# jinbeizame007/pytorch-r2d2-DPG

Hardware: NVIDIA H100
Metric: learner sequence-steps/sec (batch x seq_len) (higher is better)
Workload: dtype bf16x3 (fp32 operands split into bf16 hi+lo, three tensor-core passes, fp32 accumulate: ~16-bit operands)

## Files before the change

### include/r2d2_b200.h

```cpp
#ifndef R2D2_B200_H_
#define R2D2_B200_H_

#include <stddef.h>
#include <stdint.h>

#ifdef __cplusplus
extern "C" {
#endif

#define R2D2_OK 0
#define R2D2_ERR_CUDA (-1)
#define R2D2_ERR_ARG (-2)
#define R2D2_ERR_UNSUPPORTED (-3)
#define R2D2_ERR_STATE (-4)

typedef void* r2d2_stream_t;

int r2d2_version(void);
long long r2d2_launch_count(void);
const char* r2d2_arch(void);
const char* r2d2_last_error(void);
int r2d2_device_sm_count(int* out);

int r2d2_gemm_f32(int layout, int M, int N, int K, const float* A, long long lda, const float* B, long long ldb,
// ... 13 lines not shown

int r2d2_lstm_net_forward(const r2d2_net_shape* shape, const float* params, const float* obs, const float* act,
                          const float* h0, const float* c0, int T, int B, int repeat, int head_first_row,
                          float* out, float* workspace, r2d2_stream_t stream);

int r2d2_lstm_net_backward(const r2d2_net_shape* shape, const float* params, const float* obs, const float* act,
                           const float* d_out, int T, int B, int repeat, int head_first_row, float* grads,
                           float* d_act, float* workspace, r2d2_stream_t stream);

int r2d2_lstm_scan_forward(const float* gin, const float* whh, const float* h0, const float* c0, float* gates,
                           float* hs, float* cs, float* head_in, int T, int B, int H, int repeat, float* scratch,
                           r2d2_stream_t stream);
int r2d2_lstm_scan_backward(const float* gates, const float* hs, const float* cs, const float* whh,
                            const float* dh_head, int head_first_step, float* dgates, float* dgin, int T, int B,
                            int H, int repeat, float* scratch, r2d2_stream_t stream);

int r2d2_set_gemm_impl(int impl);
int r2d2_get_gemm_impl(void);
int r2d2_set_scan_impl(int impl);
int r2d2_get_scan_impl(void);
int r2d2_scan_status(int* status, r2d2_stream_t stream);

int r2d2_td_priority(const float* q, const float* q_next, const float* rew, const float* term, int L, int B,
                     int A, int burn_in, int n_step, float gamma, float eta, float* target, float* dq,
                     float* td_sq, float* priority, float* critic_loss, r2d2_stream_t stream);
int r2d2_td_priority_weighted(const float* q, const float* q_next, const float* rew, const float* term,
                              const float* is_weight, int L, int B, int A, int burn_in, int n_step, float gamma, float eta,
                              float* target, float* dq, float* td_sq, float* priority, float* critic_loss,
                              r2d2_stream_t stream);

#define R2D2_RESCALE_REFERENCE 0
#define R2D2_RESCALE_INVERTIBLE 1
#define R2D2_PRIORITY_SQUARED 0
#define R2D2_PRIORITY_ABS 1
typedef struct {
// ... 189 lines not shown
```

### pytorch-r2d2-dpg_b200/csrc/api.cu

```cuda
#include <atomic>
#include <cmath>

#include "common.cuh"
#include "elementwise.cuh"
#include "gemm.cuh"
#include "learner.cuh"
#include "lstm_scan.cuh"
#include "net.cuh"
#include "policy.cuh"
#include "replay.cuh"
#include "td3.cuh"

namespace r2d2 {
static thread_local std::string g_last_error;
static std::atomic<long long> g_launches{0};
void set_last_error(const std::string& msg) { g_last_error = msg; }
const char* last_error() { return g_last_error.c_str(); }
void count_launch(int n) { g_launches.fetch_add(n, std::memory_order_relaxed); }
long long launch_count() { return g_launches.load(std::memory_order_relaxed); }
int num_sms() {
  static std::atomic<int> cache[64];
  int dev = 0;
  if (cudaGetDevice(&dev) != cudaSuccess || dev < 0 || dev >= 64) return 132;
  int n = cache[dev].load(std::memory_order_relaxed);
// ... 99 lines not shown
  ScanFwdParams p;
  p.gin = gin; p.whh = whh; p.h0 = h0; p.c0 = c0; p.gates = gates; p.hs = hs; p.cs = cs; p.head_in = head_in;
  p.T = T; p.B = B; p.H = H; p.repeat = repeat; p.scratch = scratch;
  return lstm_scan_forward(p, S(stream));
}

int r2d2_lstm_scan_backward(const float* gates, const float* hs, const float* cs, const float* whh,
                            const float* dh_head, int head_first_step, float* dgates, float* dgin, int T, int B,
                            int H, int repeat, float* scratch, r2d2_stream_t stream) {
  ScanBwdParams p;
  p.gates = gates; p.hs = hs; p.cs = cs; p.whh = whh; p.dh_head = dh_head; p.head_first_step = head_first_step;
  p.dgates = dgates; p.dgin = dgin; p.T = T; p.B = B; p.H = H; p.repeat = repeat; p.scratch = scratch;
  return lstm_scan_backward(p, S(stream));
}

int r2d2_set_gemm_impl(int impl) {
  gemm_set_impl(impl != 0);
  gemm_set_impl_skinny_mma(impl != 2);
  return R2D2_OK;
}
int r2d2_get_gemm_impl(void) { return gemm_get_impl(); }
int r2d2_set_scan_impl(int impl) { lstm_scan_set_impl(impl); return R2D2_OK; }
int r2d2_get_scan_impl(void) { return lstm_scan_get_impl(); }
int r2d2_scan_status(int* status, r2d2_stream_t stream) { return lstm_scan_error_status(status, S(stream)); }

int r2d2_td_priority(const float* q, const float* q_next, const float* rew, const float* term, int L, int B,
                     int A, int burn_in, int n_step, float gamma, float eta, float* target, float* dq,
                     float* td_sq, float* priority, float* critic_loss, r2d2_stream_t stream) {
  TdPriorityParams p;
  p.q = q; p.q_next = q_next; p.rew = rew; p.term = term; p.target = target; p.dq = dq; p.td_sq = td_sq;
  p.priority = priority; p.loss_sum = critic_loss; p.L = L; p.B = B; p.A = A; p.burn_in = burn_in; p.n_step = n_step;
  p.gamma_n = (float)pow((double)gamma, (double)n_step);
  p.eta = eta;
  return td_priority(p, S(stream));
}

int r2d2_td_priority_weighted(const float* q, const float* q_next, const float* rew, const float* term,
                              const float* is_weight, int L, int B, int A, int burn_in, int n_step, float gamma, float eta,
// ... 367 lines not shown
```

### pytorch-r2d2-dpg_b200/csrc/learner.cu

```cuda
#include "learner.cuh"

#include <cmath>
#include <stdlib.h>

#include "elementwise.cuh"
#include "gemm.cuh"
#include "lstm_scan.cuh"
#include "td3.cuh"

namespace r2d2 {

static size_t align64(size_t n) { return (n + 63) & ~(size_t)63; }

int learner_create(Learner** out, const r2d2_learner_config* cfg, bool twin_critic) {
  R2D2_REQUIRE(out && cfg, "null");
  R2D2_REQUIRE(cfg->obs_size > 0 && cfg->n_actions > 0 && cfg->hidden > 0 && cfg->hidden % 4 == 0, "sizes");
  R2D2_REQUIRE(cfg->batch > 0 && cfg->burn_in >= 0 && cfg->learning > 0 && cfg->n_step > 0, "window");
  R2D2_REQUIRE(cfg->learning >= 2, "learning >= 2: the [b:-1:B] priority series of the last batch element drops its "
                                   "last TD step, so a one-step window leaves it empty");
  R2D2_REQUIRE(cfg->actor_params && cfg->critic_params && cfg->target_actor_params && cfg->target_critic_params,
               "parameter buffers");
  R2D2_REQUIRE(cfg->actor_grads && cfg->critic_grads && cfg->actor_exp_avg && cfg->actor_exp_avg_sq &&
                   cfg->critic_exp_avg && cfg->critic_exp_avg_sq, "gradient / Adam buffers");
  Learner* l = new Learner();
  l->cfg = *cfg;
  l->actor_sh = NetShape{cfg->obs_size, cfg->n_actions, cfg->hidden, false};
  l->critic_sh = NetShape{cfg->obs_size, cfg->n_actions, cfg->hidden, true};
  const int B = cfg->batch, Bn = cfg->burn_in, L = cfg->learning, n = cfg->n_step;
  const int O = cfg->obs_size, A = cfg->n_actions, H = cfg->hidden;
  const int Tt = Bn + n + L, Tc = Bn + L, Tw = Bn + L + n;
  l->rows = Tw;
  size_t total = 0;
  const size_t n_obs = align64((size_t)Tw * B * O), n_act = align64((size_t)Tw * B * A), n_rt = align64((size_t)Tw * B);
  const size_t n_states = align64((size_t)8 * B * H), n_lba = align64((size_t)L * B * A);
  const size_t n_acttc = align64((size_t)Tt * B * A);
  total += 2 * (n_obs + n_act + 2 * n_rt + n_states + align64(B)  + align64(2 * (size_t)B) );
  total += n_acttc + 8 * n_lba + align64((size_t)L * B) + align64(B) + 64;
  const size_t ws_ta = ChainWs::floats(l->actor_sh, Tt, B, 1), ws_tc = ChainWs::floats(l->critic_sh, Tt, B, 1);
  const size_t ws_c1 = ChainWs::floats(l->critic_sh, Tc, B, 1), ws_a1 = ChainWs::floats(l->actor_sh, L, B, 2);
  const size_t ws_c2 = ChainWs::floats(l->critic_sh, L, B, 1);
  total += ws_ta + ws_tc + ws_c1 + ws_a1 + ws_c2;
  total += 2 * align64(B);
  total += align64(8) + align64(4 * (size_t)kGradNormBlocks);
  l->twin = twin_critic;
  if (twin_critic) {
    l->twin_floats = align64(ws_tc) + align64(ws_c1) + 3 * n_lba + align64((size_t)L * B);
    total += l->twin_floats;
  }
  R2D2_CUDA_TRY(cudaMalloc(&l->arena, total * sizeof(float)));
  R2D2_CUDA_TRY(cudaMemset(l->arena, 0, total * sizeof(float)));
  l->arena_floats = total;
  float* p = l->arena;
  auto take = [&](size_t nfl) { float* r = p; p += align64(nfl); return r; };
  for (auto& b : l->slots) {
    b.obs = take(n_obs); b.act = take(n_act); b.rew = take(n_rt); b.term = take(n_rt);
    b.states = take(n_states); b.uniforms = take(B);
    b.leaf_idx = reinterpret_cast<long long*>(take(2 * (size_t)B));
  }
  learner_select_batch(l, 0);
  l->act_tc = take(n_acttc);
  l->q = take(n_lba); l->q_next = take(n_lba); l->target = take(n_lba); l->dq = take(n_lba);
  l->mu = take(n_lba); l->q_pi = take(n_lba); l->dq_pi = take(n_lba); l->dpre_actor = take(n_lba);
  l->td_sq = take((size_t)L * B); l->priority = take(B); l->losses = take(64);
  l->ws_ta = ChainWs::carve(take(ws_ta), l->actor_sh, Tt, B, 1);
  l->ws_tc = ChainWs::carve(take(ws_tc), l->critic_sh, Tt, B, 1);
  l->ws_c1 = ChainWs::carve(take(ws_c1), l->critic_sh, Tc, B, 1);
  l->ws_a1 = ChainWs::carve(take(ws_a1), l->actor_sh, L, B, 2);
  l->ws_c2 = ChainWs::carve(take(ws_c2), l->critic_sh, L, B, 1);
  l->ws_ta.inference_only = true;
  l->ws_tc.inference_only = true;
  for (auto& b : l->slots) {
    b.is_weight = take(B);
    R2D2_TRY(fill_f32(b.is_weight, B, 1.0f, 0));
  }
  l->optim = take(8);
  l->norm_ticket = reinterpret_cast<unsigned int*>(l->optim + 4);
  l->norm_part = reinterpret_cast<double*>(take(4 * (size_t)kGradNormBlocks));
  if (twin_critic) {
    l->ws_tc_2 = ChainWs::carve(take(ws_tc), l->critic_sh, Tt, B, 1);
    l->ws_c1_2 = ChainWs::carve(take(ws_c1), l->critic_sh, Tc, B, 1);
    l->ws_tc_2.inference_only = true;
    l->q_next2 = take(n_lba); l->q2 = take(n_lba); l->dq2 = take(n_lba);
    l->td_sq2 = take((size_t)L * B);
  }
  R2D2_CUDA_TRY(cudaStreamSynchronize(0));
  learner_select_batch(l, 0);
  {
    const char* e = getenv("R2D2_OVERLAP_INPUTS");
    l->overlap_inputs = !(e && e[0] == '0');
    if (l->overlap_inputs) {
      int lo = 0, hi = 0;
      R2D2_CUDA_TRY(cudaDeviceGetStreamPriorityRange(&lo, &hi));
      R2D2_CUDA_TRY(cudaStreamCreateWithPriority(&l->side, cudaStreamNonBlocking, lo));
      R2D2_CUDA_TRY(cudaEventCreateWithFlags(&l->ev_fork, cudaEventDisableTiming));
      R2D2_CUDA_TRY(cudaEventCreateWithFlags(&l->ev_c1_inputs, cudaEventDisableTiming));
// ... 270 lines not shown
```

### pytorch-r2d2-dpg_b200/csrc/lstm_scan.cu

```cuda
#include <cooperative_groups.h>
#include <stdlib.h>

#include "gemm.cuh"
#include "lstm_scan.cuh"
#include "elementwise.cuh"
#include "sm90.cuh"

namespace cg = cooperative_groups;

namespace r2d2 {
namespace {

constexpr int SCAN_THREADS = 256;
constexpr int UNITS_PER_CTA = 32;
constexpr int ROWS_PER_CTA = 128;
constexpr int GT_LD = ROWS_PER_CTA + 4;
constexpr int DG_LD = ROWS_PER_CTA + 8;
constexpr unsigned long long kWaitLimitNs = 4000000000ull;

__device__ unsigned g_scan_status = 0;

__device__ __forceinline__ float accurate_sigmoid(float x) { return 1.0f / (1.0f + expf(-x)); }

__device__ __forceinline__ unsigned long long global_ns() {
// ... 3 lines not shown
}

__device__ __forceinline__ void wait_slice(uint64_t* bar, uint32_t parity) {
  if (sm90::mbar_try_wait(bar, parity)) return;
  if (*reinterpret_cast<volatile unsigned*>(&g_scan_status)) return;
  const unsigned long long t0 = global_ns();
  while (!sm90::mbar_try_wait(bar, parity)) {
    if (global_ns() - t0 > kWaitLimitNs) {
      atomicExch(&g_scan_status, 1u);
      return;
    }
  }
}

__device__ __forceinline__ uint32_t slice_parity(int s) { return (uint32_t)((s - 1) >> 1) & 1u; }

template <int H> __host__ __device__ constexpr bool w_hi_in_smem() { return H > 256; }

template <int H, int NB>
struct FwdSmem {
  static constexpr int C = H / 32;
  static constexpr int HROW = UNITS_PER_CTA + 8;
  static constexpr int SLICE = 2 * NB * HROW;
  static constexpr int W_BYTES = w_hi_in_smem<H>() ? (H / 16) * 8 * 32 * 16 : 0;
  static constexpr int HB_ELEMS = 2 * C * SLICE;
  static constexpr int GT_ELEMS = NB * GT_LD;
  static constexpr int HS_ELEMS = SLICE;
  static constexpr int BAR_OFF = W_BYTES + HB_ELEMS * 2 + GT_ELEMS * 4 + HS_ELEMS * 2;
  static constexpr int BYTES = BAR_OFF + 2 * C * 8;
  static_assert((SLICE * 2) % 16 == 0 && BAR_OFF % 16 == 0, "bulk copies need 16-byte granules");
// ... 184 lines not shown
  static constexpr int C = H / 32;
  static constexpr int DG_ELEMS = 2 * NB * DG_LD;
  static constexpr int PS_LD = NB + 2;
  static constexpr int PS_ELEMS = 2 * C * UNITS_PER_CTA * PS_LD;
  static constexpr int PS_BYTES_PER_SRC = UNITS_PER_CTA * NB * 4;
  static constexpr int MT = (H / 16 + 7) / 8;
  static constexpr int W_BYTES = w_hi_in_smem<H>() ? MT * 8 * 8 * 32 * 16 : 0;
  static constexpr int STAGE_PLANES = 6;
  static constexpr int STAGE_ELEMS = STAGE_PLANES * NB * UNITS_PER_CTA;
  static constexpr int BAR_OFF = W_BYTES + DG_ELEMS * 2 + PS_ELEMS * 4 + STAGE_ELEMS * 4;
  static constexpr int BYTES = BAR_OFF + 2 * C * 8;
  static_assert(BAR_OFF % 8 == 0, "mbarrier alignment");
  static_assert(BYTES <= 232448, "BPTT scan tile does not fit in 227 KB of shared memory");
};

template <int H, int NB>
__global__ void __launch_bounds__(SCAN_THREADS, 1) lstm_scan_bwd_kernel(ScanBwdParams p) {
  constexpr int C = H / 32, NT = NB / 8;
  constexpr int M_TILES = H / 16;
  constexpr int MT = (M_TILES + 7) / 8;
  constexpr int KS = ROWS_PER_CTA / 16;
  constexpr bool WS = w_hi_in_smem<H>();
  constexpr int MG = WS ? 1 : MT;
  using SM = BwdSmem<H, NB>;
  cg::cluster_group cluster = cg::this_cluster();
  const int rank = (int)cluster.block_rank();
  const int b0 = (blockIdx.x / C) * NB;
  const int tid = threadIdx.x, lane = tid & 31, w = tid >> 5;
  const int g = lane >> 2, c = lane & 3;
  const int B = p.B, S = p.T * p.repeat;

  extern __shared__ __align__(16) unsigned char smem_raw[];
// ... 91 lines not shown
#pragma unroll
      for (int src = 0; src < C; ++src) {
        wait_slice(bar + buf * C + src, parity);
        const float* pr = ps + ((buf * C + src) * UNITS_PER_CTA + lane) * SM::PS_LD + w;
#pragma unroll
        for (int e = 0; e < NT; ++e) dh_rec[e] += pr[8 * e];
      }
    }
    sm90::cp_async_wait_all();

#pragma unroll
    for (int e = 0; e < NT; ++e) {
      const int n = w + 8 * e, b = b0 + n;
      float dg[4] = {0.f, 0.f, 0.f, 0.f};
      if (b < B) {
        const float* st = stage + n * UNITS_PER_CTA + lane;
        float dh = dh_rec[e];
        if (has_head) dh += st[5 * PLANE];
        const float ig = st[0], fg = st[PLANE], gg = st[2 * PLANE], og = st[3 * PLANE];
        const float c_prev = st[4 * PLANE];
        const float tc = tanhf(c_new[e]);
        c_new[e] = c_prev;
        const float dc = dcn[e] + dh * og * (1.f - tc * tc);
        dg[3] = dh * tc * og * (1.f - og);
        dg[0] = dc * gg * ig * (1.f - ig);
        dg[1] = dc * c_prev * fg * (1.f - fg);
        dg[2] = dc * ig * (1.f - gg * gg);
        dcn[e] = dc * fg;
        float* go = p.dgates + ((size_t)s * B + b) * gstride + ug;
        go[0] = dg[0]; go[H] = dg[1]; go[2 * H] = dg[2]; go[3 * H] = dg[3];
        if (p.repeat > 1) {
#pragma unroll
          for (int q = 0; q < 4; ++q) keep[e][q] += dg[q];
          if (s % p.repeat == 0) {
            float* gi = p.dgin + ((size_t)t * B + b) * gstride + ug;
#pragma unroll
            for (int q = 0; q < 4; ++q) { gi[q * H] = keep[e][q]; keep[e][q] = 0.f; }
          }
        }
      }
#pragma unroll
      for (int q = 0; q < 4; ++q) {
        __nv_bfloat16 hi, lo;
        split_bf16(dg[q], hi, lo);
        dgs[(0 * NB + n) * DG_LD + q * 32 + lane] = hi;
        dgs[(1 * NB + n) * DG_LD + q * 32 + lane] = lo;
      }
    }
    __syncthreads();
    if (it > 0 && tid < C) sm90::mbar_arrive_expect_tx(bar + buf * C + tid, SM::PS_BYTES_PER_SRC);

    if (s > 0) {
      prefetch(s - 1);
      const __nv_bfloat16* d_hi = dgs;
      const __nv_bfloat16* d_lo = dgs + NB * DG_LD;
      const uint32_t slot_bar = sm90::smem_u32(bar + (buf ^ 1) * C + rank);
#pragma unroll
      for (int i0 = 0; i0 < MT; i0 += MG) {
        float acc[MG][NT][4];
#pragma unroll
        for (int i = 0; i < MG; ++i)
#pragma unroll
          for (int nt = 0; nt < NT; ++nt)
#pragma unroll
            for (int e = 0; e < 4; ++e) acc[i][nt][e] = 0.f;
#pragma unroll
// ... 35 lines not shown
              const int owner = j >> 5, jl = j & 31;
              const uint32_t slot = sm90::map_cluster(
                  sm90::smem_u32(ps + (((buf ^ 1) * C + rank) * UNITS_PER_CTA + jl) * SM::PS_LD), owner);
              const uint32_t owner_bar = sm90::map_cluster(slot_bar, owner);
#pragma unroll
              for (int nt = 0; nt < NT; ++nt)
                sm90::st_async_f2(slot + (nt * 8 + 2 * c) * 4, acc[i][nt][2 * h2], acc[i][nt][2 * h2 + 1], owner_bar);
            }
          }
        }
      }
    }
    __syncthreads();
  }
  cluster.sync();
}

__global__ void lstm_cell_fwd_pointwise(const float* __restrict__ gpre, const float* __restrict__ c_prev,
                                        float* __restrict__ gates, float* __restrict__ h_out,
                                        float* __restrict__ c_out, float* __restrict__ head_in, int B, int H) {
  const int idx = blockIdx.x * blockDim.x + threadIdx.x;
  if (idx >= B * H) return;
  const int b = idx / H, u = idx % H;
  const float* gr = gpre + (size_t)b * 4 * H + u;
  const float ig = accurate_sigmoid(gr[0]), fg = accurate_sigmoid(gr[H]);
  const float gg = tanhf(gr[2 * H]), og = accurate_sigmoid(gr[3 * H]);
  const float cn = fg * c_prev[idx] + ig * gg;
  const float hn = og * tanhf(cn);
  float* go = gates + (size_t)b * 4 * H + u;
  go[0] = ig; go[H] = fg; go[2 * H] = gg; go[3 * H] = og;
// ... 149 lines not shown
}

template <int H>
int fwd_dispatch(const ScanFwdParams& p, cudaStream_t stream) {
  constexpr bool WIDE = !w_hi_in_smem<H>();
  constexpr int NB3 = WIDE ? 32 : 16;
  int nb = 0;
  R2D2_TRY(pick_nb<H>(p.B, lstm_scan_fwd_kernel<H, 8>, FwdSmem<H, 8>::BYTES, lstm_scan_fwd_kernel<H, 16>,
                      FwdSmem<H, 16>::BYTES, WIDE ? lstm_scan_fwd_kernel<H, NB3> : nullptr, FwdSmem<H, NB3>::BYTES, &nb));
  if (nb == 8)
    return launch_cluster(lstm_scan_fwd_kernel<H, 8>, p, H / 32, ceil_div(p.B, 8), FwdSmem<H, 8>::BYTES, stream);
  if (nb == 16)
    return launch_cluster(lstm_scan_fwd_kernel<H, 16>, p, H / 32, ceil_div(p.B, 16), FwdSmem<H, 16>::BYTES, stream);
  return launch_cluster(lstm_scan_fwd_kernel<H, NB3>, p, H / 32, ceil_div(p.B, NB3), FwdSmem<H, NB3>::BYTES, stream);
}
template <int H>
int bwd_dispatch(const ScanBwdParams& p, cudaStream_t stream) {
  constexpr bool WIDE = !w_hi_in_smem<H>();
  constexpr int NB3 = WIDE ? 32 : 16;
  int nb = 0;
  R2D2_TRY(pick_nb<H>(p.B, lstm_scan_bwd_kernel<H, 8>, BwdSmem<H, 8>::BYTES, lstm_scan_bwd_kernel<H, 16>,
                      BwdSmem<H, 16>::BYTES, WIDE ? lstm_scan_bwd_kernel<H, NB3> : nullptr, BwdSmem<H, NB3>::BYTES, &nb));
  if (nb == 8)
    return launch_cluster(lstm_scan_bwd_kernel<H, 8>, p, H / 32, ceil_div(p.B, 8), BwdSmem<H, 8>::BYTES, stream);
  if (nb == 16)
    return launch_cluster(lstm_scan_bwd_kernel<H, 16>, p, H / 32, ceil_div(p.B, 16), BwdSmem<H, 16>::BYTES, stream);
  return launch_cluster(lstm_scan_bwd_kernel<H, NB3>, p, H / 32, ceil_div(p.B, NB3), BwdSmem<H, NB3>::BYTES, stream);
}

}

bool lstm_scan_cluster_supported(int H) { return H == 32 || H == 64 || H == 128 || H == 256 || H == 512; }

static int g_scan_impl = -1;
void lstm_scan_set_impl(int impl) { g_scan_impl = impl ? 1 : 0; }
int lstm_scan_get_impl() {
  if (g_scan_impl < 0) {
    const char* e = getenv("R2D2_SCAN_IMPL");
    g_scan_impl = (e && (e[0] == 's' || e[0] == '0')) ? 0 : 1;
  }
  return g_scan_impl;
}
static bool use_cluster_kernels(int H) { return lstm_scan_cluster_supported(H) && lstm_scan_get_impl() == 1; }

int lstm_scan_error_status(int* out, cudaStream_t stream) {
  R2D2_REQUIRE(out, "null");
  unsigned v = 0;
  R2D2_CUDA_TRY(cudaMemcpyFromSymbolAsync(&v, g_scan_status, sizeof(v), 0, cudaMemcpyDeviceToHost, stream));
  R2D2_CUDA_TRY(cudaStreamSynchronize(stream));
  *out = (int)v;
  return R2D2_OK;
}

size_t lstm_scan_fwd_scratch_floats(int B, int H) { return (size_t)B * 4 * H; }
size_t lstm_scan_bwd_scratch_floats(int B, int H) { return (size_t)2 * B * H; }

int lstm_scan_forward(const ScanFwdParams& p, cudaStream_t stream) {
  R2D2_REQUIRE(p.gin && p.whh && p.gates && p.hs && p.cs, "null pointer");
// ... 1 lines not shown
  R2D2_REQUIRE(p.repeat == 1 || p.gates != p.gin, "gates must not alias gin when repeat > 1");
  if (use_cluster_kernels(p.H)) {
    switch (p.H) {
      case 32: return fwd_dispatch<32>(p, stream);
      case 64: return fwd_dispatch<64>(p, stream);
      case 128: return fwd_dispatch<128>(p, stream);
      case 256: return fwd_dispatch<256>(p, stream);
      case 512: return fwd_dispatch<512>(p, stream);
      default: break;
    }
  }
  return scan_forward_generic(p, p.scratch, stream);
}

int lstm_scan_backward(const ScanBwdParams& p, cudaStream_t stream) {
  R2D2_REQUIRE(p.gates && p.hs && p.cs && p.whh && p.dgates, "null pointer");
  R2D2_REQUIRE(p.T > 0 && p.B > 0 && p.H > 0 && p.repeat >= 1, "shape");
  R2D2_REQUIRE(p.repeat == 1 || (p.dgin && p.dgin != p.dgates), "dgin buffer required when repeat > 1");
  int rc = R2D2_OK;
  switch (use_cluster_kernels(p.H) ? p.H : 0) {
    case 32: rc = bwd_dispatch<32>(p, stream); break;
    case 64: rc = bwd_dispatch<64>(p, stream); break;
    case 128: rc = bwd_dispatch<128>(p, stream); break;
    case 256: rc = bwd_dispatch<256>(p, stream); break;
    case 512: rc = bwd_dispatch<512>(p, stream); break;
    default: rc = scan_backward_generic(p, stream); break;
  }
  R2D2_TRY(rc);
  if (p.dbias) {
    const float* src = p.repeat > 1 ? p.dgin : p.dgates;
    R2D2_TRY(colsum(src, 4 * p.H, p.T * p.B, 4 * p.H, p.dbias, p.dbias2, stream));
  }
  return R2D2_OK;
// ... 4 lines not shown
```

### pytorch-r2d2-dpg_b200/csrc/lstm_scan.cuh

```cuda
#pragma once
#include "common.cuh"

namespace r2d2 {

struct ScanFwdParams {
  const float* gin = nullptr;
  const float* whh = nullptr;
  const float* h0 = nullptr;
  const float* c0 = nullptr;
  float* gates = nullptr;
  float* hs = nullptr;
  float* cs = nullptr;
  float* head_in = nullptr;
  int T = 0, B = 0, H = 0, repeat = 1;
  float* scratch = nullptr;
  int no_save = 0;
};

struct ScanBwdParams {
  const float* gates = nullptr;
  const float* hs = nullptr;
  const float* cs = nullptr;
  const float* whh = nullptr;
  const float* dh_head = nullptr;
  int head_first_step = 0;
  float* dgates = nullptr;
  float* dgin = nullptr;
  int T = 0, B = 0, H = 0, repeat = 1;
  float* scratch = nullptr;
  float* dbias = nullptr;
  float* dbias2 = nullptr;
};

bool lstm_scan_cluster_supported(int H);
int lstm_scan_forward(const ScanFwdParams& p, cudaStream_t stream);
int lstm_scan_backward(const ScanBwdParams& p, cudaStream_t stream);
size_t lstm_scan_fwd_scratch_floats(int B, int H);
size_t lstm_scan_bwd_scratch_floats(int B, int H);

void lstm_scan_set_impl(int impl);
int lstm_scan_get_impl();
int lstm_scan_error_status(int* out, cudaStream_t stream);

}
```

### pytorch-r2d2-dpg_b200/csrc/net.cu

```cuda
#include "net.cuh"

#include "elementwise.cuh"
#include "gemm.cuh"
#include "lstm_scan.cuh"

namespace r2d2 {

static size_t align64(size_t n) { return (n + 63) & ~(size_t)63; }
static size_t pad_to(size_t n, size_t m) { return (n + m - 1) / m * m; }

size_t ChainWs::floats(const NetShape& s, int T, int B, int repeat) {
  const size_t H = s.hidden, A = s.act, S = (size_t)T * repeat, TB = (size_t)T * B;
  size_t n = 0;
  n += align64(TB * H);
  n += align64(TB * 4 * H);
  if (repeat > 1) n += align64(S * B * 4 * H);
  n += 2 * align64((S + 1) * B * H);
  n += align64(TB * H);
  n += align64(TB * H);
  n += 2 * align64(TB * A);
  n += align64(4 * H);
  size_t sc = lstm_scan_fwd_scratch_floats(B, s.hidden);
  const size_t sb = lstm_scan_bwd_scratch_floats(B, s.hidden);
  if (sb > sc) sc = sb;
  n += align64(sc + 64);
  n += align64(pad_to(TB, 128) * H);
  return n;
}

ChainWs ChainWs::carve(float* base, const NetShape& s, int T, int B, int repeat) {
  const size_t H = s.hidden, A = s.act, S = (size_t)T * repeat, TB = (size_t)T * B;
  ChainWs w;
  float* p = base;
  auto take = [&](size_t n) { float* r = p; p += align64(n); return r; };
  w.z1 = take(TB * H);
  w.gin = take(TB * 4 * H);
  w.gates = (repeat > 1) ? take(S * B * 4 * H) : w.gin;
  w.hs = take((S + 1) * B * H);
  w.cs = take((S + 1) * B * H);
  w.head_in = take(TB * H);
  w.dh_head = take(TB * H);
  w.head_out = take(TB * A);
  w.d_pre = take(TB * A);
  w.bias_sum = take(4 * H);
  size_t sc = lstm_scan_fwd_scratch_floats(B, s.hidden);
  const size_t sb = lstm_scan_bwd_scratch_floats(B, s.hidden);
  if (sb > sc) sc = sb;
  w.scratch = take(sc + 64);
  w.img_k = reinterpret_cast<unsigned char*>(take(pad_to(TB, 128) * H));
  return w;
}

int net_forward(const NetShape& s, const NetParams& P, const ChainWs& ws, const float* obs, const float* act,
                const float* h0, const float* c0, int T, int B, int repeat, cudaStream_t stream) {
  R2D2_TRY(net_forward_inputs(s, P, ws, obs, act, T, B, stream));
  return net_forward_scan(s, P, ws, h0, c0, T, B, repeat, stream);
}

int net_forward_inputs(const NetShape& s, const NetParams& P, const ChainWs& ws, const float* obs, const float* act,
                       int T, int B, cudaStream_t stream) {
  const int H = s.hidden, O = s.obs, A = s.act, I = s.in_features();
  const int M = T * B;
  R2D2_REQUIRE(!s.critic || act != nullptr, "critic needs actions");
  bool z1_img = false;
// ... 57 lines not shown
  if (G) {
    GemmParams g;
    g.A = d_pre; g.lda = A; g.B = hin; g.ldb = H; g.K = Mh;
    g.C = G->w3; g.ldc = H; g.M = A; g.N = H; g.split_k = gemm_suggest_split_k(A, H, Mh);
    g.colsum_a = G->b3;
    R2D2_TRY(gemm_f32(g, GEMM_TN, stream));
  }
  {
    GemmParams g;
    g.A = d_pre; g.lda = A; g.B = P.w3; g.ldb = H; g.K = A;
    g.C = ws.dh_head; g.ldc = H; g.M = Mh; g.N = H;
    if (!s.critic) { g.Z = hin; g.ldz = H; g.epilogue = EPI_MUL_DTANH; }
    R2D2_TRY(gemm_f32(g, GEMM_NN, stream));
  }
  float* dgin = (repeat > 1) ? ws.gin : ws.gates;
  {
    ScanBwdParams bp;
    bp.gates = ws.gates; bp.hs = ws.hs; bp.cs = ws.cs; bp.whh = P.whh;
    bp.dh_head = ws.dh_head; bp.head_first_step = first_row * repeat;
    bp.dgates = ws.gates; bp.dgin = dgin;
    bp.T = T; bp.B = B; bp.H = H; bp.repeat = repeat; bp.scratch = ws.scratch;
    if (G) { bp.dbias = G->bih; bp.dbias2 = G->bhh; }
    R2D2_TRY(lstm_scan_backward(bp, stream));
  }
  if (G) {
    {
      GemmParams g;
      g.A = ws.gates; g.lda = 4 * H; g.B = ws.hs; g.ldb = H; g.K = S * B;
      g.C = G->whh; g.ldc = H; g.M = 4 * H; g.N = H; g.split_k = gemm_suggest_split_k(4 * H, H, S * B);
      R2D2_TRY(gemm_f32(g, GEMM_TN, stream));
    }
    {
      GemmParams g;
      g.A = dgin; g.lda = 4 * H; g.B = ws.z1; g.ldb = H; g.K = M;
      g.C = G->wih; g.ldc = H; g.M = 4 * H; g.N = H; g.split_k = gemm_suggest_split_k(4 * H, H, M);
      g.reuse_packed_a = (repeat == 1);
      R2D2_TRY(gemm_f32(g, GEMM_TN, stream));
    }
  }
  {
    GemmParams g;
    g.A = dgin; g.lda = 4 * H; g.B = P.wih; g.ldb = H; g.K = 4 * H;
    g.C = ws.z1; g.ldc = H; g.M = M; g.N = H; g.Z = ws.z1; g.ldz = H; g.epilogue = EPI_MUL_DTANH;
    R2D2_TRY(gemm_f32(g, GEMM_NN, stream));
  }
  if (G) {
    GemmParams g;
    g.A = ws.z1; g.lda = H; g.B = obs; g.ldb = O; g.K = M;
    g.C = G->w1; g.ldc = I; g.M = H; g.N = O; g.split_k = gemm_suggest_split_k(H, O, M);
    g.colsum_a = G->b1;
    R2D2_TRY(gemm_f32(g, GEMM_TN, stream));
    if (s.critic) {
      GemmParams g2 = g;
      g2.colsum_a = nullptr;
      g2.B = act; g2.ldb = A; g2.C = G->w1 + O; g2.N = A; g2.split_k = gemm_suggest_split_k(H, A, M);
      R2D2_TRY(gemm_f32(g2, GEMM_TN, stream));
    }
  }
// ... 13 lines not shown
```

### pytorch-r2d2-dpg_b200/csrc/net.cuh

```cuda
#pragma once
#include "common.cuh"

namespace r2d2 {

struct NetShape {
  int obs = 0, act = 0, hidden = 0;
  bool critic = false;
  int in_features() const { return obs + (critic ? act : 0); }
  size_t param_count() const {
    const size_t H = hidden, I = in_features(), A = act;
    return H * I + H + 4 * H * H * 2 + 4 * H * 2 + A * H + A;
  }
};

struct NetParams {
  float *w1, *b1, *wih, *whh, *bih, *bhh, *w3, *b3;
  static NetParams from_flat(float* flat, const NetShape& s) {
    const size_t H = s.hidden, I = s.in_features(), A = s.act;
    NetParams p;
    p.w1 = flat;            p.b1 = p.w1 + H * I;
    p.wih = p.b1 + H;       p.whh = p.wih + 4 * H * H;
    p.bih = p.whh + 4 * H * H; p.bhh = p.bih + 4 * H;
    p.w3 = p.bhh + 4 * H;   p.b3 = p.w3 + A * H;
    return p;
  }
};

struct ChainWs {
  float* z1 = nullptr;
  float* gin = nullptr;
  float* gates = nullptr;
  float* hs = nullptr;
  float* cs = nullptr;
  float* head_in = nullptr;
  float* dh_head = nullptr;
  float* head_out = nullptr;
  float* d_pre = nullptr;
  float* bias_sum = nullptr;
  float* scratch = nullptr;
  unsigned char* img_k = nullptr;
  bool inference_only = false;
  static size_t floats(const NetShape& s, int T, int B, int repeat);
  static ChainWs carve(float* base, const NetShape& s, int T, int B, int repeat);
};

int net_forward(const NetShape& s, const NetParams& P, const ChainWs& ws, const float* obs, const float* act,
                const float* h0, const float* c0, int T, int B, int repeat, cudaStream_t stream);
int net_forward_inputs(const NetShape& s, const NetParams& P, const ChainWs& ws, const float* obs, const float* act,
                       int T, int B, cudaStream_t stream);
int net_forward_scan(const NetShape& s, const NetParams& P, const ChainWs& ws, const float* h0, const float* c0, int T,
                     int B, int repeat, cudaStream_t stream);
int net_head_forward(const NetShape& s, const NetParams& P, const ChainWs& ws, int first_row, int T, int B,
                     int repeat, float* out, long long ldo, cudaStream_t stream);
int net_backward(const NetShape& s, const NetParams& P, const NetParams* G, const ChainWs& ws, const float* obs,
                 const float* act, const float* d_pre, int first_row, int T, int B, int repeat, float* d_act,
                 const float* dact_z, cudaStream_t stream);

}
// ... 1 lines not shown
```

### pytorch-r2d2-dpg_b200/r2d2_b200/native.py

```python
from __future__ import annotations

import ctypes
import os
from ctypes import (POINTER, Structure, byref, c_char_p, c_double, c_float, c_int, c_longlong, c_size_t, c_uint,
                    c_ulonglong, c_void_p)

import numpy as np
import torch

_HERE = os.path.dirname(os.path.abspath(__file__))
LIB_PATH = os.environ.get("R2D2_B200_LIB") or os.path.join(os.path.dirname(_HERE), "libr2d2_b200.so")

GEMM_NT, GEMM_NN, GEMM_TN = 0, 1, 2
EPI_NONE, EPI_TANH, EPI_MUL_DTANH, EPI_ADD_Z = 0, 1, 2, 3


class NativeError(RuntimeError):
    pass


class NetShape(Structure):
    _fields_ = [("obs_size", c_int), ("n_actions", c_int), ("hidden", c_int), ("is_critic", c_int)]


# ... 66 lines not shown
    "r2d2_last_error": (c_char_p, []),
    "r2d2_device_sm_count": (c_int, [POINTER(c_int)]),
    "r2d2_gemm_f32": (c_int, [c_int, c_int, c_int, c_int, c_void_p, c_longlong, c_void_p, c_longlong, c_void_p,
                              c_longlong, c_void_p, c_longlong, c_int, c_void_p, c_longlong, c_void_p, c_void_p,
                              c_longlong, c_int, c_int, c_void_p]),
    "r2d2_net_param_count": (c_size_t, [POINTER(NetShape)]),
    "r2d2_net_workspace_floats": (c_size_t, [POINTER(NetShape), c_int, c_int, c_int]),
    "r2d2_lstm_net_forward": (c_int, [POINTER(NetShape), c_void_p, c_void_p, c_void_p, c_void_p, c_void_p, c_int,
                                      c_int, c_int, c_int, c_void_p, c_void_p, c_void_p]),
    "r2d2_lstm_net_backward": (c_int, [POINTER(NetShape), c_void_p, c_void_p, c_void_p, c_void_p, c_int, c_int,
                                       c_int, c_int, c_void_p, c_void_p, c_void_p, c_void_p]),
    "r2d2_lstm_scan_forward": (c_int, [c_void_p, c_void_p, c_void_p, c_void_p, c_void_p, c_void_p, c_void_p, c_void_p,
                                       c_int, c_int, c_int, c_int, c_void_p, c_void_p]),
    "r2d2_lstm_scan_backward": (c_int, [c_void_p, c_void_p, c_void_p, c_void_p, c_void_p, c_int, c_void_p, c_void_p,
                                        c_int, c_int, c_int, c_int, c_void_p, c_void_p]),
    "r2d2_set_gemm_impl": (c_int, [c_int]),
    "r2d2_get_gemm_impl": (c_int, []),
    "r2d2_set_scan_impl": (c_int, [c_int]),
    "r2d2_get_scan_impl": (c_int, []),
    "r2d2_scan_status": (c_int, [POINTER(c_int), c_void_p]),
    "r2d2_td_priority": (c_int, [c_void_p, c_void_p, c_void_p, c_void_p, c_int, c_int, c_int, c_int, c_int, c_float,
                                 c_float, c_void_p, c_void_p, c_void_p, c_void_p, c_void_p, c_void_p]),
    "r2d2_td_priority_weighted": (c_int, [c_void_p, c_void_p, c_void_p, c_void_p, c_void_p, c_int, c_int, c_int, c_int,
                                          c_int, c_float, c_float, c_void_p, c_void_p, c_void_p, c_void_p, c_void_p,
                                          c_void_p]),
    "r2d2_td_priority_ex": (c_int, [c_void_p, c_void_p, c_void_p, c_void_p, c_void_p, c_int, c_int, c_int, c_int, c_int,
                                    c_float, c_float, c_void_p, c_void_p, c_void_p, c_void_p, c_void_p,
                                    POINTER(TdOptions), c_void_p]),
    "r2d2_nstep_rewards": (c_int, [c_void_p, c_void_p, c_int, c_int, c_int, c_float, c_void_p, c_void_p]),
    "r2d2_actor_priorities": (c_int, [c_void_p, c_void_p, c_void_p, c_void_p, c_void_p, c_int, c_int, c_int, c_int, c_int,
                                      c_float, c_float, c_int, c_void_p, c_void_p]),
    "r2d2_actor_priorities_ex": (c_int, [c_void_p, c_void_p, c_void_p, c_void_p, c_void_p, c_int, c_int, c_int, c_int,
                                         c_int, c_float, c_float, c_int, c_void_p, POINTER(TdOptions), c_void_p]),
    "r2d2_policy_workspace_floats": (c_size_t, [POINTER(NetShape), c_int]),
# ... 132 lines not shown
```

Before: 1.158 million.

## Emit pre-split bf16 operand images from LSTM backward scan for downstream GEMMs

The backward LSTM scan kernel now writes the gate gradients directly as bf16 hi/lo tiled operand images (MN- and K-major) that the following weight-gradient and data-gradient GEMMs read in place of packing fp32 dG themselves. When images are used, the fp32 dgates store can be skipped. This is meant to remove the separate pack/split passes and the fp32 round trips between the scan and the GEMMs. The cost is extra stores and a block sync inside the serial scan loop, plus larger workspace.

```diff
diff --git a/include/r2d2_b200.h b/include/r2d2_b200.h
--- a/include/r2d2_b200.h
+++ b/include/r2d2_b200.h
@@ -51,11 +51,17 @@
 int r2d2_lstm_scan_backward(const float* gates, const float* hs, const float* cs, const float* whh,
                             const float* dh_head, int head_first_step, float* dgates, float* dgin, int T, int B,
                             int H, int repeat, float* scratch, r2d2_stream_t stream);
+int r2d2_lstm_scan_backward_images(const float* gates, const float* hs, const float* cs, const float* whh,
+                                   const float* dh_head, int head_first_step, float* dgates, float* dgin, int T, int B,
+                                   int H, int repeat, unsigned char* dg_img_mn, unsigned char* dgin_img_mn,
+                                   unsigned char* dgin_img_k, int no_dgates, r2d2_stream_t stream);
 
 int r2d2_set_gemm_impl(int impl);
 int r2d2_get_gemm_impl(void);
 int r2d2_set_scan_impl(int impl);
 int r2d2_get_scan_impl(void);
+int r2d2_set_scan_operand_images(int on);
+int r2d2_scan_emits_operand_images(int H, int B);
 int r2d2_scan_status(int* status, r2d2_stream_t stream);
 
 int r2d2_td_priority(const float* q, const float* q_next, const float* rew, const float* term, int L, int B,
diff --git a/pytorch-r2d2-dpg_b200/csrc/api.cu b/pytorch-r2d2-dpg_b200/csrc/api.cu
--- a/pytorch-r2d2-dpg_b200/csrc/api.cu
+++ b/pytorch-r2d2-dpg_b200/csrc/api.cu
@@ -137,6 +137,17 @@
   return lstm_scan_backward(p, S(stream));
 }
 
+int r2d2_lstm_scan_backward_images(const float* gates, const float* hs, const float* cs, const float* whh,
+                                   const float* dh_head, int head_first_step, float* dgates, float* dgin, int T, int B,
+                                   int H, int repeat, unsigned char* dg_img_mn, unsigned char* dgin_img_mn,
+                                   unsigned char* dgin_img_k, int no_dgates, r2d2_stream_t stream) {
+  ScanBwdImageParams p;
+  p.gates = gates; p.hs = hs; p.cs = cs; p.whh = whh; p.dh_head = dh_head; p.head_first_step = head_first_step;
+  p.dgates = dgates; p.dgin = dgin; p.T = T; p.B = B; p.H = H; p.repeat = repeat;
+  p.dg_img_mn = dg_img_mn; p.dgin_img_mn = dgin_img_mn; p.dgin_img_k = dgin_img_k; p.no_dgates = no_dgates;
+  return lstm_scan_backward(p, S(stream));
+}
+
 int r2d2_set_gemm_impl(int impl) {
   gemm_set_impl(impl != 0);
   gemm_set_impl_skinny_mma(impl != 2);
@@ -145,6 +156,8 @@
 int r2d2_get_gemm_impl(void) { return gemm_get_impl(); }
 int r2d2_set_scan_impl(int impl) { lstm_scan_set_impl(impl); return R2D2_OK; }
 int r2d2_get_scan_impl(void) { return lstm_scan_get_impl(); }
+int r2d2_set_scan_operand_images(int on) { lstm_scan_set_operand_images(on); return R2D2_OK; }
+int r2d2_scan_emits_operand_images(int H, int B) { return lstm_scan_emits_operand_images(H, B) ? 1 : 0; }
 int r2d2_scan_status(int* status, r2d2_stream_t stream) { return lstm_scan_error_status(status, S(stream)); }
 
 int r2d2_td_priority(const float* q, const float* q_next, const float* rew, const float* term, int L, int B,
diff --git a/pytorch-r2d2-dpg_b200/csrc/learner.cu b/pytorch-r2d2-dpg_b200/csrc/learner.cu
--- a/pytorch-r2d2-dpg_b200/csrc/learner.cu
+++ b/pytorch-r2d2-dpg_b200/csrc/learner.cu
@@ -37,8 +37,11 @@
   total += 2 * (n_obs + n_act + 2 * n_rt + n_states + align64(B)  + align64(2 * (size_t)B) );
   total += n_acttc + 8 * n_lba + align64((size_t)L * B) + align64(B) + 64;
   const size_t ws_ta = ChainWs::floats(l->actor_sh, Tt, B, 1), ws_tc = ChainWs::floats(l->critic_sh, Tt, B, 1);
-  const size_t ws_c1 = ChainWs::floats(l->critic_sh, Tc, B, 1), ws_a1 = ChainWs::floats(l->actor_sh, L, B, 2);
-  const size_t ws_c2 = ChainWs::floats(l->critic_sh, L, B, 1);
+  const bool img = lstm_scan_emits_operand_images(H, B);
+  const ChainBwd wgrad = img ? ChainBwd::wgrad : ChainBwd::none, dgrad = img ? ChainBwd::dgrad : ChainBwd::none;
+  const size_t ws_c1 = ChainWs::floats(l->critic_sh, Tc, B, 1, wgrad);
+  const size_t ws_a1 = ChainWs::floats(l->actor_sh, L, B, 2, wgrad);
+  const size_t ws_c2 = ChainWs::floats(l->critic_sh, L, B, 1, dgrad);
   total += ws_ta + ws_tc + ws_c1 + ws_a1 + ws_c2;
   total += 2 * align64(B);
   total += align64(8) + align64(4 * (size_t)kGradNormBlocks);
@@ -64,9 +67,9 @@
   l->td_sq = take((size_t)L * B); l->priority = take(B); l->losses = take(64);
   l->ws_ta = ChainWs::carve(take(ws_ta), l->actor_sh, Tt, B, 1);
   l->ws_tc = ChainWs::carve(take(ws_tc), l->critic_sh, Tt, B, 1);
-  l->ws_c1 = ChainWs::carve(take(ws_c1), l->critic_sh, Tc, B, 1);
-  l->ws_a1 = ChainWs::carve(take(ws_a1), l->actor_sh, L, B, 2);
-  l->ws_c2 = ChainWs::carve(take(ws_c2), l->critic_sh, L, B, 1);
+  l->ws_c1 = ChainWs::carve(take(ws_c1), l->critic_sh, Tc, B, 1, wgrad);
+  l->ws_a1 = ChainWs::carve(take(ws_a1), l->actor_sh, L, B, 2, wgrad);
+  l->ws_c2 = ChainWs::carve(take(ws_c2), l->critic_sh, L, B, 1, dgrad);
   l->ws_ta.inference_only = true;
   l->ws_tc.inference_only = true;
   for (auto& b : l->slots) {
@@ -78,7 +81,7 @@
   l->norm_part = reinterpret_cast<double*>(take(4 * (size_t)kGradNormBlocks));
   if (twin_critic) {
     l->ws_tc_2 = ChainWs::carve(take(ws_tc), l->critic_sh, Tt, B, 1);
-    l->ws_c1_2 = ChainWs::carve(take(ws_c1), l->critic_sh, Tc, B, 1);
+    l->ws_c1_2 = ChainWs::carve(take(ws_c1), l->critic_sh, Tc, B, 1, wgrad);
     l->ws_tc_2.inference_only = true;
     l->q_next2 = take(n_lba); l->q2 = take(n_lba); l->dq2 = take(n_lba);
     l->td_sq2 = take((size_t)L * B);
diff --git a/pytorch-r2d2-dpg_b200/csrc/lstm_scan.cu b/pytorch-r2d2-dpg_b200/csrc/lstm_scan.cu
--- a/pytorch-r2d2-dpg_b200/csrc/lstm_scan.cu
+++ b/pytorch-r2d2-dpg_b200/csrc/lstm_scan.cu
@@ -1,5 +1,7 @@
 #include <cooperative_groups.h>
 #include <stdlib.h>
+
+#include <type_traits>
 
 #include "gemm.cuh"
 #include "lstm_scan.cuh"
@@ -41,6 +43,20 @@
 }
 
 __device__ __forceinline__ uint32_t slice_parity(int s) { return (uint32_t)((s - 1) >> 1) & 1u; }
+
+constexpr int IMG_PLANE_BYTES = 8192, IMG_TILE_BYTES = 16384;
+__device__ __forceinline__ size_t img_mn_offset(size_t r, int c, int k_tiles) {
+  return ((size_t)(c >> 7) * k_tiles + (r >> 5)) * IMG_TILE_BYTES +
+         (((((int)r & 31) >> 3) * 128) + ((c & 127) >> 3) * 8 + ((int)r & 7)) * 16;
+}
+__device__ __forceinline__ size_t img_k_offset(size_t r, int c, int k_tiles) {
+  return ((r >> 7) * k_tiles + (c >> 5)) * IMG_TILE_BYTES +
+         (((((int)r & 127) >> 3) * 32) + ((c & 31) >> 3) * 8 + ((int)r & 7)) * 16;
+}
+__device__ __forceinline__ void store_piece(unsigned char* img, size_t off, uint4 hi, uint4 lo) {
+  *reinterpret_cast<uint4*>(img + off) = hi;
+  *reinterpret_cast<uint4*>(img + off + IMG_PLANE_BYTES) = lo;
+}
 
 template <int H> __host__ __device__ constexpr bool w_hi_in_smem() { return H > 256; }
 
@@ -255,8 +271,16 @@
   static_assert(BYTES <= 232448, "BPTT scan tile does not fit in 227 KB of shared memory");
 };
 
-template <int H, int NB>
-__global__ void __launch_bounds__(SCAN_THREADS, 1) lstm_scan_bwd_kernel(ScanBwdParams p) {
+struct BwdImageKernelParams : ScanBwdImageParams {
+  int kt_dg = 0, kt_dgin = 0;
+};
+
+__device__ __forceinline__ bool stores_dgates(const ScanBwdParams&) { return true; }
+__device__ __forceinline__ bool stores_dgates(const BwdImageKernelParams& p) { return !p.no_dgates; }
+
+template <int H, int NB, typename P>
+__device__ __forceinline__ void scan_bwd(P p) {
+  constexpr bool IMG = std::is_same<P, BwdImageKernelParams>::value;
   constexpr int C = H / 32, NT = NB / 8;
   constexpr int M_TILES = H / 16;
   constexpr int MT = (M_TILES + 7) / 8;
@@ -378,7 +402,7 @@
       const int n = w + 8 * e, b = b0 + n;
       float dg[4] = {0.f, 0.f, 0.f, 0.f};
       if (b < B) {
-        const float* st = stage + n * UNITS_PER_CTA + lane;
+        float* st = stage + n * UNITS_PER_CTA + lane;
         float dh = dh_rec[e];
         if (has_head) dh += st[5 * PLANE];
         const float ig = st[0], fg = st[PLANE], gg = st[2 * PLANE], og = st[3 * PLANE];
@@ -391,15 +415,21 @@
         dg[1] = dc * c_prev * fg * (1.f - fg);
         dg[2] = dc * ig * (1.f - gg * gg);
         dcn[e] = dc * fg;
-        float* go = p.dgates + ((size_t)s * B + b) * gstride + ug;
-        go[0] = dg[0]; go[H] = dg[1]; go[2 * H] = dg[2]; go[3 * H] = dg[3];
+        if (stores_dgates(p)) {
+          float* go = p.dgates + ((size_t)s * B + b) * gstride + ug;
+          go[0] = dg[0]; go[H] = dg[1]; go[2 * H] = dg[2]; go[3 * H] = dg[3];
+        }
         if (p.repeat > 1) {
 #pragma unroll
           for (int q = 0; q < 4; ++q) keep[e][q] += dg[q];
           if (s % p.repeat == 0) {
             float* gi = p.dgin + ((size_t)t * B + b) * gstride + ug;
 #pragma unroll
-            for (int q = 0; q < 4; ++q) { gi[q * H] = keep[e][q]; keep[e][q] = 0.f; }
+            for (int q = 0; q < 4; ++q) {
+              gi[q * H] = keep[e][q];
+              if constexpr (IMG) st[q * PLANE] = keep[e][q];
+              keep[e][q] = 0.f;
+            }
           }
         }
       }
@@ -414,6 +444,59 @@
     __syncthreads();
     if (it > 0 && tid < C) sm90::mbar_arrive_expect_tx(bar + buf * C + tid, SM::PS_BYTES_PER_SRC);
 
+    constexpr int PIECES = NB * 4 * (UNITS_PER_CTA / 8);
+    if constexpr (IMG) {
+      if (p.repeat > 1 && s % p.repeat == 0) {
+        const size_t r0 = (size_t)t * B;
+        constexpr int PER_THREAD = (PIECES + SCAN_THREADS - 1) / SCAN_THREADS;
+        float4 v[PER_THREAD][2];
+#pragma unroll
+        for (int k = 0; k < PER_THREAD; ++k) {
+          const int idx = tid + k * SCAN_THREADS, n = idx % NB, j = (idx / NB) % 4, q = idx / (4 * NB);
+          if (idx < PIECES && b0 + n < B) {
+            const float4* src = reinterpret_cast<const float4*>(stage + q * PLANE + n * UNITS_PER_CTA + 8 * j);
+            v[k][0] = src[0];
+            v[k][1] = src[1];
+          }
+        }
+        __syncthreads();
+#pragma unroll
+        for (int k = 0; k < PER_THREAD; ++k) {
+          const int idx = tid + k * SCAN_THREADS, n = idx % NB, j = (idx / NB) % 4, q = idx / (4 * NB), b = b0 + n;
+          if (idx < PIECES && b < B) {
+            uint4 hi, lo;
+            split_pack2(v[k][0].x, v[k][0].y, hi.x, lo.x);
+            split_pack2(v[k][0].z, v[k][0].w, hi.y, lo.y);
+            split_pack2(v[k][1].x, v[k][1].y, hi.z, lo.z);
+            split_pack2(v[k][1].z, v[k][1].w, hi.w, lo.w);
+            const int col = q * H + rank * UNITS_PER_CTA + 8 * j;
+            if (p.dgin_img_mn) store_piece(p.dgin_img_mn, img_mn_offset(r0 + b, col, p.kt_dgin), hi, lo);
+            if (p.dgin_img_k) store_piece(p.dgin_img_k, img_k_offset(r0 + b, col, H / 8), hi, lo);
+          }
+        }
+      }
+    }
+
+    if constexpr (IMG) {
+      const size_t r0 = (size_t)s * B;
+      unsigned tv;
+      asm volatile("mov.u32 %0, %%tid.x;" : "=r"(tv));
+#pragma unroll
+      for (int idx = (int)tv; idx < PIECES; idx += SCAN_THREADS) {
+        const int n = idx % NB, j = (idx / NB) % 4, q = idx / (4 * NB), b = b0 + n;
+        if (b < B) {
+          const __nv_bfloat16* src = dgs + n * DG_LD + q * UNITS_PER_CTA + 8 * j;
+          const uint4 hi = *reinterpret_cast<const uint4*>(src);
+          const uint4 lo = *reinterpret_cast<const uint4*>(src + NB * DG_LD);
+          const int col = q * H + rank * UNITS_PER_CTA + 8 * j;
+          if (p.dg_img_mn) store_piece(p.dg_img_mn, img_mn_offset(r0 + b, col, p.kt_dg), hi, lo);
+          if (p.repeat == 1) {
+            if (p.dgin_img_mn) store_piece(p.dgin_img_mn, img_mn_offset(r0 + b, col, p.kt_dg), hi, lo);
+            if (p.dgin_img_k) store_piece(p.dgin_img_k, img_k_offset(r0 + b, col, H / 8), hi, lo);
+          }
+        }
+      }
+    }
     if (s > 0) {
       prefetch(s - 1);
       const __nv_bfloat16* d_hi = dgs;
@@ -479,6 +562,13 @@
     __syncthreads();
   }
   cluster.sync();
+}
+
+template <int H, int NB>
+__global__ void __launch_bounds__(SCAN_THREADS, 1) lstm_scan_bwd_kernel(ScanBwdParams p) { scan_bwd<H, NB>(p); }
+template <int H, int NB>
+__global__ void __launch_bounds__(SCAN_THREADS, 1) lstm_scan_bwd_images_kernel(BwdImageKernelParams p) {
+  scan_bwd<H, NB>(p);
 }
 
 __global__ void lstm_cell_fwd_pointwise(const float* __restrict__ gpre, const float* __restrict__ c_prev,
@@ -658,18 +748,30 @@
     return launch_cluster(lstm_scan_fwd_kernel<H, 16>, p, H / 32, ceil_div(p.B, 16), FwdSmem<H, 16>::BYTES, stream);
   return launch_cluster(lstm_scan_fwd_kernel<H, NB3>, p, H / 32, ceil_div(p.B, NB3), FwdSmem<H, NB3>::BYTES, stream);
 }
-template <int H>
-int bwd_dispatch(const ScanBwdParams& p, cudaStream_t stream) {
+template <int H, typename P, typename K8, typename K16, typename K32>
+int bwd_launch(const P& p, K8 k8, K16 k16, K32 k32, cudaStream_t stream) {
   constexpr bool WIDE = !w_hi_in_smem<H>();
   constexpr int NB3 = WIDE ? 32 : 16;
   int nb = 0;
-  R2D2_TRY(pick_nb<H>(p.B, lstm_scan_bwd_kernel<H, 8>, BwdSmem<H, 8>::BYTES, lstm_scan_bwd_kernel<H, 16>,
-                      BwdSmem<H, 16>::BYTES, WIDE ? lstm_scan_bwd_kernel<H, NB3> : nullptr, BwdSmem<H, NB3>::BYTES, &nb));
-  if (nb == 8)
-    return launch_cluster(lstm_scan_bwd_kernel<H, 8>, p, H / 32, ceil_div(p.B, 8), BwdSmem<H, 8>::BYTES, stream);
-  if (nb == 16)
-    return launch_cluster(lstm_scan_bwd_kernel<H, 16>, p, H / 32, ceil_div(p.B, 16), BwdSmem<H, 16>::BYTES, stream);
-  return launch_cluster(lstm_scan_bwd_kernel<H, NB3>, p, H / 32, ceil_div(p.B, NB3), BwdSmem<H, NB3>::BYTES, stream);
+  R2D2_TRY(pick_nb<H>(p.B, k8, BwdSmem<H, 8>::BYTES, k16, BwdSmem<H, 16>::BYTES, WIDE ? k32 : nullptr,
+                      BwdSmem<H, NB3>::BYTES, &nb));
+  if (nb == 8) return launch_cluster(k8, p, H / 32, ceil_div(p.B, 8), BwdSmem<H, 8>::BYTES, stream);
+  if (nb == 16) return launch_cluster(k16, p, H / 32, ceil_div(p.B, 16), BwdSmem<H, 16>::BYTES, stream);
+  return launch_cluster(k32, p, H / 32, ceil_div(p.B, NB3), BwdSmem<H, NB3>::BYTES, stream);
+}
+template <int H>
+int bwd_dispatch(const ScanBwdImageParams& p, cudaStream_t stream) {
+  constexpr int NB3 = w_hi_in_smem<H>() ? 16 : 32;
+  if (!(p.dg_img_mn || p.dgin_img_mn || p.dgin_img_k)) {
+    return bwd_launch<H>(static_cast<const ScanBwdParams&>(p), lstm_scan_bwd_kernel<H, 8>, lstm_scan_bwd_kernel<H, 16>,
+                         lstm_scan_bwd_kernel<H, NB3>, stream);
+  }
+  BwdImageKernelParams q;
+  static_cast<ScanBwdImageParams&>(q) = p;
+  q.kt_dg = (int)ceil_div_ll((long long)p.T * p.repeat * p.B, 32);
+  q.kt_dgin = (int)ceil_div_ll((long long)p.T * p.B, 32);
+  return bwd_launch<H>(q, lstm_scan_bwd_images_kernel<H, 8>, lstm_scan_bwd_images_kernel<H, 16>,
+                       lstm_scan_bwd_images_kernel<H, NB3>, stream);
 }
 
 }
@@ -686,6 +788,12 @@
   return g_scan_impl;
 }
 static bool use_cluster_kernels(int H) { return lstm_scan_cluster_supported(H) && lstm_scan_get_impl() == 1; }
+
+static int g_scan_images = 1;
+void lstm_scan_set_operand_images(int on) { g_scan_images = on ? 1 : 0; }
+bool lstm_scan_emits_operand_images(int H, int B) {
+  return g_scan_images && use_cluster_kernels(H) && (long long)B * H >= 16384;
+}
 
 int lstm_scan_error_status(int* out, cudaStream_t stream) {
   R2D2_REQUIRE(out, "null");
@@ -717,9 +825,19 @@
 }
 
 int lstm_scan_backward(const ScanBwdParams& p, cudaStream_t stream) {
+  ScanBwdImageParams q;
+  static_cast<ScanBwdParams&>(q) = p;
+  return lstm_scan_backward(q, stream);
+}
+
+int lstm_scan_backward(const ScanBwdImageParams& p, cudaStream_t stream) {
   R2D2_REQUIRE(p.gates && p.hs && p.cs && p.whh && p.dgates, "null pointer");
   R2D2_REQUIRE(p.T > 0 && p.B > 0 && p.H > 0 && p.repeat >= 1, "shape");
   R2D2_REQUIRE(p.repeat == 1 || (p.dgin && p.dgin != p.dgates), "dgin buffer required when repeat > 1");
+  const bool img = p.dg_img_mn || p.dgin_img_mn || p.dgin_img_k;
+  R2D2_REQUIRE(!img || use_cluster_kernels(p.H), "operand images from a scan route that does not write them");
+  R2D2_REQUIRE(!p.no_dgates || (img && !(p.dbias && p.repeat == 1)),
+               "no_dgates: image mode only, and the bias sums read the fp32 dG at repeat 1");
   int rc = R2D2_OK;
   switch (use_cluster_kernels(p.H) ? p.H : 0) {
     case 32: rc = bwd_dispatch<32>(p, stream); break;
diff --git a/pytorch-r2d2-dpg_b200/csrc/lstm_scan.cuh b/pytorch-r2d2-dpg_b200/csrc/lstm_scan.cuh
--- a/pytorch-r2d2-dpg_b200/csrc/lstm_scan.cuh
+++ b/pytorch-r2d2-dpg_b200/csrc/lstm_scan.cuh
@@ -32,14 +32,24 @@
   float* dbias2 = nullptr;
 };
 
+struct ScanBwdImageParams : ScanBwdParams {
+  unsigned char* dg_img_mn = nullptr;
+  unsigned char* dgin_img_mn = nullptr;
+  unsigned char* dgin_img_k = nullptr;
+  int no_dgates = 0;
+};
+
 bool lstm_scan_cluster_supported(int H);
 int lstm_scan_forward(const ScanFwdParams& p, cudaStream_t stream);
 int lstm_scan_backward(const ScanBwdParams& p, cudaStream_t stream);
+int lstm_scan_backward(const ScanBwdImageParams& p, cudaStream_t stream);
 size_t lstm_scan_fwd_scratch_floats(int B, int H);
 size_t lstm_scan_bwd_scratch_floats(int B, int H);
 
 void lstm_scan_set_impl(int impl);
 int lstm_scan_get_impl();
+bool lstm_scan_emits_operand_images(int H, int B);
+void lstm_scan_set_operand_images(int on);
 int lstm_scan_error_status(int* out, cudaStream_t stream);
 
 }
diff --git a/pytorch-r2d2-dpg_b200/csrc/net.cu b/pytorch-r2d2-dpg_b200/csrc/net.cu
--- a/pytorch-r2d2-dpg_b200/csrc/net.cu
+++ b/pytorch-r2d2-dpg_b200/csrc/net.cu
@@ -6,10 +6,14 @@
 
 namespace r2d2 {
 
+static bool gemm_reads_operand_images(int M, int N, int K) {
+  return gemm_get_impl() == 1 && (!gemm_get_impl_skinny_mma() || (M > 32 && N > 32 && K >= 64));
+}
+
 static size_t align64(size_t n) { return (n + 63) & ~(size_t)63; }
 static size_t pad_to(size_t n, size_t m) { return (n + m - 1) / m * m; }
 
-size_t ChainWs::floats(const NetShape& s, int T, int B, int repeat) {
+size_t ChainWs::floats(const NetShape& s, int T, int B, int repeat, ChainBwd bwd) {
   const size_t H = s.hidden, A = s.act, S = (size_t)T * repeat, TB = (size_t)T * B;
   size_t n = 0;
   n += align64(TB * H);
@@ -25,10 +29,15 @@
   if (sb > sc) sc = sb;
   n += align64(sc + 64);
   n += align64(pad_to(TB, 128) * H);
+  if (bwd != ChainBwd::none) n += align64(pad_to(TB, 128) * 4 * H);
+  if (bwd == ChainBwd::wgrad) {
+    n += align64(pad_to(S * B, 128) * 4 * H);
+    if (repeat > 1) n += align64(pad_to(TB, 128) * 4 * H);
+  }
   return n;
 }
 
-ChainWs ChainWs::carve(float* base, const NetShape& s, int T, int B, int repeat) {
+ChainWs ChainWs::carve(float* base, const NetShape& s, int T, int B, int repeat, ChainBwd bwd) {
   const size_t H = s.hidden, A = s.act, S = (size_t)T * repeat, TB = (size_t)T * B;
   ChainWs w;
   float* p = base;
@@ -48,6 +57,12 @@
   if (sb > sc) sc = sb;
   w.scratch = take(sc + 64);
   w.img_k = reinterpret_cast<unsigned char*>(take(pad_to(TB, 128) * H));
+  auto take_img = [&](size_t rows) { return reinterpret_cast<unsigned char*>(take(pad_to(rows, 128) * 4 * H)); };
+  if (bwd != ChainBwd::none) w.dgin_img_k = take_img(TB);
+  if (bwd == ChainBwd::wgrad) {
+    w.dg_img_mn = take_img(S * B);
+    if (repeat > 1) w.dgin_img_mn = take_img(TB);
+  }
   return w;
 }
 
@@ -135,13 +150,24 @@
     R2D2_TRY(gemm_f32(g, GEMM_NN, stream));
   }
   float* dgin = (repeat > 1) ? ws.gin : ws.gates;
-  {
-    ScanBwdParams bp;
+  const bool images = ws.dgin_img_k && (!G || ws.dg_img_mn) && lstm_scan_emits_operand_images(H, B) &&
+                      gemm_reads_operand_images(M, H, 4 * H) &&
+                      (!G || (gemm_reads_operand_images(4 * H, H, S * B) && gemm_reads_operand_images(4 * H, H, M)));
+  {
+    ScanBwdImageParams bp;
     bp.gates = ws.gates; bp.hs = ws.hs; bp.cs = ws.cs; bp.whh = P.whh;
     bp.dh_head = ws.dh_head; bp.head_first_step = first_row * repeat;
     bp.dgates = ws.gates; bp.dgin = dgin;
     bp.T = T; bp.B = B; bp.H = H; bp.repeat = repeat; bp.scratch = ws.scratch;
     if (G) { bp.dbias = G->bih; bp.dbias2 = G->bhh; }
+    if (images) {
+      bp.dgin_img_k = ws.dgin_img_k;
+      if (G) {
+        bp.dg_img_mn = ws.dg_img_mn;
+        if (repeat > 1) bp.dgin_img_mn = ws.dgin_img_mn;
+      }
+      bp.no_dgates = (repeat > 1 || !G) ? 1 : 0;
+    }
     R2D2_TRY(lstm_scan_backward(bp, stream));
   }
   if (G) {
@@ -149,13 +175,15 @@
       GemmParams g;
       g.A = ws.gates; g.lda = 4 * H; g.B = ws.hs; g.ldb = H; g.K = S * B;
       g.C = G->whh; g.ldc = H; g.M = 4 * H; g.N = H; g.split_k = gemm_suggest_split_k(4 * H, H, S * B);
+      if (images) g.A_img = ws.dg_img_mn;
       R2D2_TRY(gemm_f32(g, GEMM_TN, stream));
     }
     {
       GemmParams g;
       g.A = dgin; g.lda = 4 * H; g.B = ws.z1; g.ldb = H; g.K = M;
       g.C = G->wih; g.ldc = H; g.M = 4 * H; g.N = H; g.split_k = gemm_suggest_split_k(4 * H, H, M);
-      g.reuse_packed_a = (repeat == 1);
+      if (images) g.A_img = (repeat > 1) ? ws.dgin_img_mn : ws.dg_img_mn;
+      else g.reuse_packed_a = (repeat == 1);
       R2D2_TRY(gemm_f32(g, GEMM_TN, stream));
     }
   }
@@ -163,6 +191,7 @@
     GemmParams g;
     g.A = dgin; g.lda = 4 * H; g.B = P.wih; g.ldb = H; g.K = 4 * H;
     g.C = ws.z1; g.ldc = H; g.M = M; g.N = H; g.Z = ws.z1; g.ldz = H; g.epilogue = EPI_MUL_DTANH;
+    if (images) g.A_img = ws.dgin_img_k;
     R2D2_TRY(gemm_f32(g, GEMM_NN, stream));
   }
   if (G) {
diff --git a/pytorch-r2d2-dpg_b200/csrc/net.cuh b/pytorch-r2d2-dpg_b200/csrc/net.cuh
--- a/pytorch-r2d2-dpg_b200/csrc/net.cuh
+++ b/pytorch-r2d2-dpg_b200/csrc/net.cuh
@@ -26,6 +26,8 @@
   }
 };
 
+enum class ChainBwd { none, dgrad, wgrad };
+
 struct ChainWs {
   float* z1 = nullptr;
   float* gin = nullptr;
@@ -39,9 +41,12 @@
   float* bias_sum = nullptr;
   float* scratch = nullptr;
   unsigned char* img_k = nullptr;
+  unsigned char* dg_img_mn = nullptr;
+  unsigned char* dgin_img_mn = nullptr;
+  unsigned char* dgin_img_k = nullptr;
   bool inference_only = false;
-  static size_t floats(const NetShape& s, int T, int B, int repeat);
-  static ChainWs carve(float* base, const NetShape& s, int T, int B, int repeat);
+  static size_t floats(const NetShape& s, int T, int B, int repeat, ChainBwd bwd = ChainBwd::none);
+  static ChainWs carve(float* base, const NetShape& s, int T, int B, int repeat, ChainBwd bwd = ChainBwd::none);
 };
 
 int net_forward(const NetShape& s, const NetParams& P, const ChainWs& ws, const float* obs, const float* act,
diff --git a/pytorch-r2d2-dpg_b200/r2d2_b200/native.py b/pytorch-r2d2-dpg_b200/r2d2_b200/native.py
--- a/pytorch-r2d2-dpg_b200/r2d2_b200/native.py
+++ b/pytorch-r2d2-dpg_b200/r2d2_b200/native.py
@@ -104,10 +104,15 @@
                                        c_int, c_int, c_int, c_int, c_void_p, c_void_p]),
     "r2d2_lstm_scan_backward": (c_int, [c_void_p, c_void_p, c_void_p, c_void_p, c_void_p, c_int, c_void_p, c_void_p,
                                         c_int, c_int, c_int, c_int, c_void_p, c_void_p]),
+    "r2d2_lstm_scan_backward_images": (c_int, [c_void_p, c_void_p, c_void_p, c_void_p, c_void_p, c_int, c_void_p,
+                                               c_void_p, c_int, c_int, c_int, c_int, c_void_p, c_void_p, c_void_p,
+                                               c_int, c_void_p]),
     "r2d2_set_gemm_impl": (c_int, [c_int]),
     "r2d2_get_gemm_impl": (c_int, []),
     "r2d2_set_scan_impl": (c_int, [c_int]),
     "r2d2_get_scan_impl": (c_int, []),
+    "r2d2_set_scan_operand_images": (c_int, [c_int]),
+    "r2d2_scan_emits_operand_images": (c_int, [c_int, c_int]),
     "r2d2_scan_status": (c_int, [POINTER(c_int), c_void_p]),
     "r2d2_td_priority": (c_int, [c_void_p, c_void_p, c_void_p, c_void_p, c_int, c_int, c_int, c_int, c_int, c_float,
                                  c_float, c_void_p, c_void_p, c_void_p, c_void_p, c_void_p, c_void_p]),
```

Result: faster. 1.192 million, median of 6 (+2.9%).
